# georghess/neurad-studio

Measured on AMD Instinct MI355X. Metric: ray-samples/sec (4096 rays x 128 samples), higher is better.
Workload: dtype f32; 1 GPU; BASELINE config[1]: NeuRAD hash-grid (16 levels, T=2^19, F=2, fp32) + 64-wide MLPs, 4096 rays x 128 samples per GPU, PowerSampler bins + ray ordering pass + fused field + compositing (forward / render path); rays_per_gpu=4096, samples_per_ray=128, parallelism=rays sharded x1, no collective

## Files before the change

### neurad_studio_amd/csrc/render.hip

```cpp
#include "common.h"
#include "render_variants.h"

namespace nrhip {

struct FieldDev {
  GridDev grid;
  const void* table;
  float scale;
  const float* gw0; const float* gb0;
  const float* gw1; const float* gb1;
  const float* fw0; const float* fb0;
  const float* fw1; const float* fb1;
  const float* fw2; const float* fb2;
  int use_sdf;
  float beta;
  uint32_t lay[NRHIP_MAX_LEVELS * 4];
};

struct SaveDev {
  float* enc;
  float* hg;
  float* xf;
  float* hf;
};
// ... 152 lines not shown
    d16[blk * 8 + 4 + v] = (unsigned short)(m >> 16);
    d16[NBLK * KB * 64 * 8 + blk * 4 + v] = (unsigned short)(l >> 16);
  }
}

using f16x8 = __attribute__((ext_vector_type(8))) _Float16;
using f16x2 = __attribute__((ext_vector_type(2))) _Float16;
using f32x2 = __attribute__((ext_vector_type(2))) float;
constexpr float kPairAct = 64.f, kPairW = 128.f, kPairFit = 65000.f;
constexpr bool kPairsDefault = true;

template <bool CHAIN, int NBLK, int KQ>
__device__ __forceinline__ float pair_src(const float* __restrict__ W, int ldw, int row_off, int e) {
  const int t = e & 7, lane = (e >> 3) & 63, rest = e >> 9;
  const int q = rest % KQ, mb = rest / KQ;
  const int i = lane & 15, g = lane >> 4;
  const int col = CHAIN ? (16 * (2 * q + (t >> 2)) + 4 * g + (t & 3)) : (8 * g + t);
  return W[(size_t)(row_off + 16 * mb + i) * ldw + col];
}
__device__ __forceinline__ bool pair_store(float* __restrict__ region, int N, int e, float w) {
  _Float16* d16 = reinterpret_cast<_Float16*>(region);
  const float ws = w * kPairW;
  const _Float16 h = (_Float16)ws;
  d16[e] = h;
  d16[N + e] = (_Float16)(ws - (float)h);
  return !(fabsf(ws) < kPairFit);
}

template <bool CHAIN, int NBLK, int KQ>
__device__ __forceinline__ void mfma_layer_pairs(const float* __restrict__ wf, const float* __restrict__ W, int ldw,
                                                 int row_off, bool wbad, int lane, const float (&b)[8 * KQ],
                                                 f32x4 (&acc)[NBLK]) {
  float mx = 0.f;
#pragma unroll
  for (int k = 0; k < 8 * KQ; ++k) mx = fmaxf(mx, fabsf(b[k]));
  if (__builtin_expect(wbad || __builtin_amdgcn_ballot_w64(!(mx < kPairFit)) != 0ull, 0)) {
    int opaque = 0;
    asm volatile("" : "+v"(opaque));
    const int g = lane >> 4;
    const float* Wl = W + (size_t)(row_off + (lane & 15)) * ldw + opaque;
#pragma unroll
    for (int s = 0; s < 8 * KQ; ++s) {
      const int col = CHAIN ? (16 * (s >> 2) + 4 * g + (s & 3)) : (8 * g + s);
#pragma unroll
      for (int mb = 0; mb < NBLK; ++mb)
        acc[mb] = __builtin_amdgcn_mfma_f32_16x16x4f32(Wl[(size_t)16 * mb * ldw + col] * kPairW, b[s], acc[mb], 0, 0, 0);
    }
  } else {
    const f16x8* w8 = reinterpret_cast<const f16x8*>(wf);
    constexpr int LO = NBLK * KQ * 64;
#pragma unroll
    for (int q = 0; q < KQ; ++q) {
      f16x8 xh, xl;
#pragma unroll
      for (int k = 0; k < 8; k += 2) {
        const f32x2 v = {b[8 * q + k], b[8 * q + k + 1]};
        const f16x2 h = __builtin_convertvector(v, f16x2);
        const f16x2 l = __builtin_convertvector(v - __builtin_convertvector(h, f32x2), f16x2);
        xh[k] = h[0], xh[k + 1] = h[1], xl[k] = l[0], xl[k + 1] = l[1];
      }
#pragma unroll
      for (int mb = 0; mb < NBLK; ++mb)
        acc[mb] = __builtin_amdgcn_mfma_f32_16x16x32_f16(w8[(mb * KQ + q) * 64 + lane], xh, acc[mb], 0, 0, 0);
#pragma unroll
      for (int mb = 0; mb < NBLK; ++mb)
        acc[mb] = __builtin_amdgcn_mfma_f32_16x16x32_f16(w8[LO + (mb * KQ + q) * 64 + lane], xh, acc[mb], 0, 0, 0);
#pragma unroll
      for (int mb = 0; mb < NBLK; ++mb)
        acc[mb] = __builtin_amdgcn_mfma_f32_16x16x32_f16(w8[(mb * KQ + q) * 64 + lane], xl, acc[mb], 0, 0, 0);
    }
  }
#pragma unroll
  for (int mb = 0; mb < NBLK; ++mb) acc[mb] *= 1.f / kPairW;
}

template <Prod PROD, bool CHAIN, int NBLK, int K>
__device__ __forceinline__ void tile_layer(const float* __restrict__ wf, const float* __restrict__ W, int ldw, int row_off,
                                           bool wbad, int lane, const float (&b)[K], f32x4 (&acc)[NBLK]) {
  if constexpr (PROD == Prod::F16Pairs) mfma_layer_pairs<CHAIN, NBLK, K / 8>(wf, W, ldw, row_off, wbad, lane, b, acc);
  else if constexpr (PROD == Prod::Bf16Split) mfma_layer_split<NBLK, K / 4>(wf, lane, b, acc);
  else mfma_layer<NBLK, K>(wf, lane, b, acc);
}

template <int L, int F, int H, Prod PROD = Prod::F32>
__device__ __forceinline__ void stage_field_weights(const FieldDev& fd, float* __restrict__ lds) {
  using Ld = Lds<H, PROD>;
  constexpr int LF = EncFrame<L, F>::LF;
  static_assert(PROD == Prod::F32 || EncFrame<L, F>::FULL, "split / pair products: L * F == 32 only");
  constexpr int NB = H / 16;
  constexpr int T = 256;
  constexpr int N_G0 = H * 32 / T, N_G1 = 32 * H / T, N_F0 = H * 32 / T, N_F1 = H * H / T, N_F2 = 32 * H / T,
                N_SH = 16 * H / T;
  static_assert((H * 32) % T == 0 && (H * H) % T == 0 && (16 * H) % T == 0, "regions are whole passes of the block");
  const int tid = threadIdx.x;
  float vg0[N_G0], vg1[N_G1], vf0[N_F0], vf1[N_F1], vf2[N_F2], vsh[N_SH], vs[7];
  if constexpr (PROD == Prod::Bf16Split) {
    stage_split_matrix<false, NB, 2>(lds + Ld::G0, fd.gw0, LF, 0);
    stage_split_matrix<true, 2, NB>(lds + Ld::G1, fd.gw1, H, 1);
    stage_split_matrix<true, NB, 2>(lds + Ld::F0, fd.fw0, 48, 0);
    stage_split_matrix<true, NB, NB>(lds + Ld::F1, fd.fw1, H, 0);
  } else if constexpr (PROD == Prod::F16Pairs) {
    static_assert(H % 32 == 0, "fp16 pairs: K = 32 steps");
    if (tid == 0) reinterpret_cast<int*>(lds)[Ld::FLG] = 0;
    __syncthreads();
#pragma unroll
    for (int it = 0; it < N_G0; ++it) vg0[it] = pair_src<false, NB, 1>(fd.gw0, LF, 0, it * T + tid);
#pragma unroll
    for (int it = 0; it < N_G1; ++it) vg1[it] = pair_src<true, 2, H / 32>(fd.gw1, H, 1, it * T + tid);
#pragma unroll
    for (int it = 0; it < N_F0; ++it) vf0[it] = pair_src<true, NB, 1>(fd.fw0, 48, 0, it * T + tid);
#pragma unroll
    for (int it = 0; it < N_F1; ++it) vf1[it] = pair_src<true, NB, H / 32>(fd.fw1, H, 0, it * T + tid);
  } else {
#pragma unroll
    for (int it = 0; it < N_G0; ++it) vg0[it] = enc_frag_src<L, F, NB>(fd.gw0, it * T + tid);
#pragma unroll
    for (int it = 0; it < N_G1; ++it) vg1[it] = frag_src<true, 2, H / 4>(fd.gw1, H, 1, it * T + tid);
#pragma unroll
    for (int it = 0; it < N_F0; ++it) vf0[it] = frag_src<true, NB, 8>(fd.fw0, 48, 0, it * T + tid);
#pragma unroll
    for (int it = 0; it < N_F1; ++it) vf1[it] = frag_src<true, NB, H / 4>(fd.fw1, H, 0, it * T + tid);
  }
#pragma unroll
  for (int it = 0; it < N_F2; ++it) vf2[it] = frag_src<true, 2, H / 4>(fd.fw2, H, 0, it * T + tid);
#pragma unroll
  for (int it = 0; it < N_SH; ++it) {
    const int e = it * T + tid, c = e / H, n = e - c * H;
    vsh[it] = fd.fw0[(size_t)n * 48 + 32 + c];
  }
  const int th = tid < H ? tid : 0, t33 = tid < 33 ? tid : 0, t32 = tid & 31;
  vs[0] = fd.gw1[th];
  vs[1] = fd.gb0 ? fd.gb0[th] : 0.f;
  vs[2] = fd.fb0 ? fd.fb0[th] : 0.f;
  vs[3] = fd.fb1 ? fd.fb1[th] : 0.f;
  vs[4] = fd.gb1 ? fd.gb1[t33] : 0.f;
  vs[5] = fd.fb2 ? fd.fb2[t32] : 0.f;
  vs[6] = fd.grid.scal[t32];
  if constexpr (PROD == Prod::F16Pairs) {
    constexpr float kB = kPairAct * kPairW;
    vs[0] *= 1.f / kPairAct, vs[1] *= kB, vs[2] *= kB, vs[3] *= kB;
    if (t33 != 0) vs[4] *= kB;
#pragma unroll
    for (int it = 0; it < N_F2; ++it) vf2[it] *= 1.f / kPairAct;
#pragma unroll
    for (int it = 0; it < N_SH; ++it) vsh[it] *= kB;
    bool bad = false;
#pragma unroll
    for (int it = 0; it < N_G0; ++it) bad |= pair_store(lds + Ld::G0, H * 32, it * T + tid, vg0[it]);
#pragma unroll
    for (int it = 0; it < N_G1; ++it) bad |= pair_store(lds + Ld::G1, 32 * H, it * T + tid, vg1[it]);
#pragma unroll
    for (int it = 0; it < N_F0; ++it) bad |= pair_store(lds + Ld::F0, H * 32, it * T + tid, vf0[it]);
#pragma unroll
    for (int it = 0; it < N_F1; ++it) bad |= pair_store(lds + Ld::F1, H * H, it * T + tid, vf1[it]);
    if (bad) reinterpret_cast<int*>(lds)[Ld::FLG] = 1;
  }
  if constexpr (PROD == Prod::F32) {
#pragma unroll
    for (int it = 0; it < N_G0; ++it) lds[Ld::G0 + it * T + tid] = vg0[it];
#pragma unroll
    for (int it = 0; it < N_G1; ++it) lds[Ld::G1 + it * T + tid] = vg1[it];
#pragma unroll
    for (int it = 0; it < N_F0; ++it) lds[Ld::F0 + it * T + tid] = vf0[it];
#pragma unroll
    for (int it = 0; it < N_F1; ++it) lds[Ld::F1 + it * T + tid] = vf1[it];
  }
#pragma unroll
  for (int it = 0; it < N_F2; ++it) lds[Ld::F2 + it * T + tid] = vf2[it];
#pragma unroll
  for (int it = 0; it < N_SH; ++it) lds[Ld::SHW + it * T + tid] = vsh[it];
  if (tid < H) {
    lds[Ld::SDFW + tid] = vs[0];
    lds[Ld::BG0 + tid] = vs[1];
    lds[Ld::BF0 + tid] = vs[2];
    lds[Ld::BF1 + tid] = vs[3];
  }
  if (tid < 33) lds[Ld::BG1 + tid] = vs[4];
  if (tid < 32) {
    lds[Ld::BF2 + tid] = vs[5];
    lds[Ld::SCAL + tid] = vs[6];
  }
}

__device__ __forceinline__ void stream_store(float* p, f32x4 v) { __builtin_nontemporal_store(v, reinterpret_cast<f32x4*>(p)); }

template <int N>
__device__ __forceinline__ float row_shr(float v, float fill) {
  return dpp_row_shr<N>(v, fill);
}
__device__ __forceinline__ float row_sum16(float v) {
  v += __shfl_xor(v, 1, 64);
  v += __shfl_xor(v, 2, 64);
  v += __shfl_xor(v, 4, 64);
  v += __shfl_xor(v, 8, 64);
  return v;
}

template <int LPL, int F>
struct TileFetch {
  float fv[LPL][8][F];
  float x, y, z, std;
  float t0, t1;
};

struct RayRange {
  int64_t end;
  int S, stride;
};

struct PendingTile {
  int64_t pos;
  int64_t ray;
  int t;
  bool valid;
  float t0, t1;
  float ox, oy, oz, dx, dy, dz, area;
  int ncand;
};

__device__ __forceinline__ float from_lane(float v, int byte_addr) {
  return __builtin_bit_cast(float, __builtin_amdgcn_ds_bpermute(byte_addr, __builtin_bit_cast(int, v)));
}
__device__ __forceinline__ void put_block(float* geo, int lane, const SamplePos& p) {
  geo[lane] = p.x, geo[64 + lane] = p.y, geo[128 + lane] = p.z, geo[192 + lane] = p.std;
}
__device__ __forceinline__ SamplePos get_block(const float* geo, int src) {
  SamplePos p;
  p.x = geo[src], p.y = geo[64 + src], p.z = geo[128 + src], p.std = geo[192 + src];
  return p;
}

template <bool ACT>
__device__ __forceinline__ void fill_block(float* geo, float* ageo, int lane, const PendingTile& pt, float scale) {
  if constexpr (ACT) {
    const SamplePos gs = sample_gaussian(pt.ox, pt.oy, pt.oz, pt.dx, pt.dy, pt.dz, pt.area, pt.t0, pt.t1);
    put_block(ageo, lane, gs);
    put_block(geo, lane, contract_gaussian(gs.x, gs.y, gs.z, gs.std, scale));
  } else {
    put_block(geo, lane, sample_position(pt.ox, pt.oy, pt.oz, pt.dx, pt.dy, pt.dz, pt.area, pt.t0, pt.t1, scale));
  }
}

__device__ __forceinline__ void load_pending(PendingTile& p, int64_t pos, int t, const RayRange& rr, int lane,
                                             const int32_t* __restrict__ order, const float* __restrict__ ro,
                                             const float* __restrict__ rd, const float* __restrict__ rarea,
                                             const float* __restrict__ rstarts, const float* __restrict__ rends,
                                             const int32_t* __restrict__ cand_count = nullptr) {
  p.pos = pos, p.t = t, p.valid = pos < rr.end;
  const int64_t pc = p.valid ? pos : rr.end - 1;
  const int64_t ray = order ? (int64_t)order[pc] : pc;
  p.ray = ray;
  const int s = p.valid ? 64 * (t >> 2) + lane : lane;
  const int64_t si = ray * rr.stride + (s < rr.S ? s : rr.S - 1);
  if ((t & 3) == 0) {
    p.t0 = rstarts[si];
    p.t1 = rends[si];
  }
  p.ox = ro[3 * ray], p.oy = ro[3 * ray + 1], p.oz = ro[3 * ray + 2];
  p.dx = rd[3 * ray], p.dy = rd[3 * ray + 1], p.dz = rd[3 * ray + 2];
  p.area = rarea[ray];
  p.ncand = cand_count ? cand_count[ray] : 0;
}

__device__ __forceinline__ void load_pending_packed(PendingTile& p, int64_t pos, int t, const RayRange& rr, int lane,
                                                    const int32_t* __restrict__ order, const float* __restrict__ ro,
                                                    const float* __restrict__ rd, const float* __restrict__ rarea,
                                                    const float* __restrict__ rstarts, const float* __restrict__ rends,
                                                    const int64_t* __restrict__ segs, int& first, int& count,
                                                    const int32_t* __restrict__ cand_count = nullptr) {
  p.pos = pos, p.t = t, p.valid = pos < rr.end;
  const int64_t pc = p.valid ? pos : rr.end - 1;
  const int64_t ray = order ? (int64_t)order[pc] : pc;
  p.ray = ray;
  const int b = (int)segs[ray], n = (int)segs[ray + 1] - b;
  first = b, count = n;
  const int s = p.valid ? 64 * (t >> 2) + lane : lane;
  int si = b + (s < n ? s : n - 1);
  si = si < 0 ? 0 : si;
  si = si < rr.S ? si : rr.S - 1;
  if ((t & 3) == 0) {
    p.t0 = rstarts[si];
    p.t1 = rends[si];
  }
  p.ox = ro[3 * ray], p.oy = ro[3 * ray + 1], p.oz = ro[3 * ray + 2];
  p.dx = rd[3 * ray], p.dy = rd[3 * ray + 1], p.dz = rd[3 * ray + 2];
  p.area = rarea[ray];
  p.ncand = cand_count ? cand_count[ray] : 0;
}

__device__ __forceinline__ void layout_corners(float x, float y, float z, float scale, uint32_t my, uint32_t mz,
                                               uint32_t mask, uint32_t (&idx)[8]) {
  const float sx = __fmul_rn(x, scale), sy = __fmul_rn(y, scale), sz = __fmul_rn(z, scale);
  const uint32_t ifx = (uint32_t)(int)floorf(sx), ify = (uint32_t)(int)floorf(sy), ifz = (uint32_t)(int)floorf(sz);
  const uint32_t icx = (uint32_t)(int)ceilf(sx), icy = (uint32_t)(int)ceilf(sy), icz = (uint32_t)(int)ceilf(sz);
  const uint32_t hyc = icy * my, hyf = ify * my, hzc = icz * mz, hzf = ifz * mz;
  idx[0] = (icx ^ hyc ^ hzc) & mask;
  idx[1] = (icx ^ hyf ^ hzc) & mask;
  idx[2] = (ifx ^ hyf ^ hzc) & mask;
  idx[3] = (ifx ^ hyc ^ hzc) & mask;
  idx[4] = (icx ^ hyc ^ hzf) & mask;
  idx[5] = (icx ^ hyf ^ hzf) & mask;
  idx[6] = (ifx ^ hyf ^ hzf) & mask;
  idx[7] = (ifx ^ hyc ^ hzf) & mask;
}

template <int L, int F, bool HALF, bool RELAY = false>
__device__ __forceinline__ void issue_tile(const FieldDev& fd, const PendingTile& pt, int g, uint32_t mask,
                                           const float* scal_lds, TileFetch<EncFrame<L, F>::LPL, F>& tf,
                                           float* geo, int lane, const uint32_t* lay_lds = nullptr) {
  constexpr int LPL = EncFrame<L, F>::LPL;
  if ((pt.t & 3) == 0) fill_block<false>(geo, nullptr, lane, pt, fd.scale);
  const int src = 16 * (pt.t & 3) + (lane & 15);
  const SamplePos p = get_block(geo, src);
  tf.t0 = from_lane(pt.t0, src << 2);
  tf.t1 = from_lane(pt.t1, src << 2);
  if (!EncFrame<L, F>::busy(g)) return;
#pragma unroll
  for (int q = 0; q < LPL; ++q) {
    if constexpr (RELAY) {
      const uint4 ly = *reinterpret_cast<const uint4*>(lay_lds + 4 * q);
      uint32_t idx[8];
      layout_corners(p.x, p.y, p.z, scal_lds[q], ly.x, ly.y, ly.z, idx);
#pragma unroll
      for (int k = 0; k < 8; ++k) Entry<F, HALF>::load(fd.table, ly.w + idx[k], tf.fv[q][k]);
    } else {
      const Corners cs = hash_corners(p.x, p.y, p.z, scal_lds[q], mask);
#pragma unroll
      for (int k = 0; k < 8; ++k)
        Entry<F, HALF>::load(fd.table, ((uint32_t)(LPL * g + q) << fd.grid.log2T) + cs.idx[k], tf.fv[q][k]);
    }
  }
}

template <int L, int F, bool HALF>
__device__ __forceinline__ void issue_tile_actors(const FieldDev& fd, const ActorFieldDev& ad, const PendingTile& pt, int g,
                                                  uint32_t mask, const float* scal_lds, const float* ascal_lds,
                                                  const int32_t* __restrict__ cand_actor,
                                                  const float* __restrict__ cand_w2b, const float* __restrict__ bounds,
                                                  const void* const* __restrict__ tables,
                                                  TileFetch<EncFrame<L, F>::LPL, F>& tf, int& slot_out,
                                                  float* geo, float* ageo, int lane) {
  constexpr int LPL = EncFrame<L, F>::LPL;
  const bool busy = EncFrame<L, F>::busy(g);
  const int n = __builtin_amdgcn_readfirstlane(pt.ncand);
  const uint32_t row = (uint32_t)__builtin_amdgcn_readfirstlane((int)((uint32_t)pt.ray * (uint32_t)ad.K));
  if ((pt.t & 3) == 0) fill_block<true>(geo, ageo, lane, pt, fd.scale);
  const int src = 16 * (pt.t & 3) + (lane & 15);
  const SamplePos gs = get_block(ageo, src), ps = get_block(geo, src);
  tf.t0 = from_lane(pt.t0, src << 2);
  tf.t1 = from_lane(pt.t1, src << 2);
  int slot = -1;
  if (n > 0) {
    for (int c = 0; c < n; ++c) {
      const float* w = cand_w2b + (row + (uint32_t)c) * 12u;
// ... 61 lines not shown
    const float nn = sqrtf(ddx * ddx + ddy * ddy + ddz * ddz) + 1e-7f;
    if (mine) bx = ddx / nn, by = ddy / nn, bz = ddz / nn;
  }
  float sh[16];
  sh4((bx + 1.f) / 2.f, (by + 1.f) / 2.f, (bz + 1.f) / 2.f, sh);
#pragma unroll
  for (int c = 0; c < 16; ++c)
    if ((c >> 2) == g) shb[c & 3] = sh[c];
}

template <int L, int F>
__device__ __forceinline__ void blend_tile_actors(const TileFetch<EncFrame<L, F>::LPL, F>& tf, int slot, int g, int La,
                                                  const float* scal_lds, const float* ascal_lds, float (&feat)[8]) {
  using EF = EncFrame<L, F>;
  constexpr int LPL = EF::LPL;
  const bool in_box = slot >= 0;
#pragma unroll
  for (int q = 0; q < LPL; ++q) {
    const int lv = LPL * g + q, alv = lv < La ? lv : La - 1;
    const float sc = in_box ? ascal_lds[alv] : scal_lds[q];
    Corners c;
    const float sx = __fmul_rn(tf.x, sc), sy = __fmul_rn(tf.y, sc), sz = __fmul_rn(tf.z, sc);
    c.ox = __fsub_rn(sx, floorf(sx)), c.oy = __fsub_rn(sy, floorf(sy)), c.oz = __fsub_rn(sz, floorf(sz));
    float v[F];
    lerp_corners<F>(c, tf.fv[q], v);
    const float rw = (in_box && lv >= La) ? 0.f : rescale_weight(sc, tf.std);
#pragma unroll
    for (int f = 0; f < F; ++f) feat[q * F + f] = EF::busy(g) ? v[f] * rw : 0.f;
  }
#pragma unroll
  for (int k = EF::W; k < 8; ++k) feat[k] = 0.f;
}

template <int L, int F>
__device__ __forceinline__ void blend_tile(const TileFetch<EncFrame<L, F>::LPL, F>& tf, const SamplePos& p, int g,
                                           const float* scal_lds, float (&feat)[8]) {
  using EF = EncFrame<L, F>;
  constexpr int LPL = EF::LPL;
#pragma unroll
  for (int q = 0; q < LPL; ++q) {
    const float sc = scal_lds[q];
    Corners c;
    const float sx = __fmul_rn(p.x, sc), sy = __fmul_rn(p.y, sc), sz = __fmul_rn(p.z, sc);
    c.ox = __fsub_rn(sx, floorf(sx)), c.oy = __fsub_rn(sy, floorf(sy)), c.oz = __fsub_rn(sz, floorf(sz));
    float v[F];
    lerp_corners<F>(c, tf.fv[q], v);
    const float rw = rescale_weight(sc, p.std);
#pragma unroll
    for (int f = 0; f < F; ++f) feat[q * F + f] = EF::busy(g) ? v[f] * rw : 0.f;
  }
#pragma unroll
  for (int k = EF::W; k < 8; ++k) feat[k] = 0.f;
}

template <int L, int F, int H, bool HALF, Out OUT, Src SRC, Prod PROD, Lay LAY = Lay::Dense>
__global__ __launch_bounds__(256, 2) void render_kernel(
    FieldDev fd, int64_t n_rays, int S, int stride, const int32_t* __restrict__ order, const float* __restrict__ ro,
    const float* __restrict__ rd, const float* __restrict__ rarea, const float* __restrict__ rstarts,
    const float* __restrict__ rends, float* __restrict__ out_feat, float* __restrict__ out_depth,
    float* __restrict__ out_acc, float* __restrict__ out_w, float* __restrict__ out_sdf, float* __restrict__ out_alpha,
    SaveDev sv, float stop_eps, const int32_t* __restrict__ range, ActorFieldDev ad,
    const int32_t* __restrict__ cand_count,
    const int32_t* __restrict__ cand_actor, const float* __restrict__ cand_w2b, const float* __restrict__ bounds,
    const void* const* __restrict__ tables) {
  using EF = EncFrame<L, F>;
  static_assert(render_variant_ok(L, F, OUT, SRC, PROD, LAY), "not a legal variant: see render_variant_ok");
  static_assert(H % 16 == 0 && H >= 16 && H <= 128, "hidden width");
  constexpr bool COMPOSITE = OUT == Out::Composite;
  constexpr bool ACT = SRC == Src::Actors, RELAY = SRC == Src::EvalTable, OVR = SRC == Src::Overrides;
  constexpr bool PAIRS = PROD == Prod::F16Pairs;
  constexpr bool PACKED = LAY != Lay::Dense;
  const int64_t* const segs = LAY == Lay::PackedActors ? reinterpret_cast<const int64_t*>(sv.enc)
                                                       : reinterpret_cast<const int64_t*>(tables);
  const int32_t* const pcand = ACT ? cand_count : nullptr;
  const int32_t* const ovr_row = cand_count;
  const float* const ovr_rows = cand_w2b;
  const float* const ovr_dirs = bounds;
  using Ld = Lds<H, PROD>;
  constexpr int NB = H / 16;
  constexpr int LPL = EF::LPL;
  constexpr bool DEFER = COMPOSITE;
  extern __shared__ __attribute__((aligned(16))) float lds[];

  stage_field_weights<L, F, H, PROD>(fd, lds);
  if constexpr (ACT || OVR) {
    for (int e = threadIdx.x; e < 16 * H; e += 256) lds[Ld::SHF + e] = frag_src<true, NB, 4>(fd.fw0 + 32, 48, 0, e);
  }
  if constexpr (ACT) {
    if (threadIdx.x < ad.La) lds[Ld::ASCAL + threadIdx.x] = ad.scal[threadIdx.x];
  }
  if constexpr (RELAY) {
    if (threadIdx.x < 4 * L) reinterpret_cast<uint32_t*>(lds + Ld::LAY)[threadIdx.x] = fd.lay[threadIdx.x];
  }
  __syncthreads();
  bool wbad = false;
  if constexpr (PAIRS) wbad = __builtin_amdgcn_readfirstlane(reinterpret_cast<const int*>(lds)[Ld::FLG]) != 0;

  const int lane = threadIdx.x & 63;
  const int wid = __builtin_amdgcn_readfirstlane(threadIdx.x >> 6);
  const int j = lane & 15, g = lane >> 4;
  const uint32_t mask = (1u << fd.grid.log2T) - 1u;
  const int ntile = (S + 15) >> 4;

  const int nx = (int)gridDim.x < 8 ? (int)gridDim.x : 8;
  const int xcd = (int)blockIdx.x % nx, lb = (int)blockIdx.x / nx;
  const int nblk = ((int)gridDim.x - xcd + nx - 1) / nx;
  const int64_t first = range ? range[0] : 0, count = range ? range[1] - range[0] : n_rays;
  const int64_t lo = first + count * xcd / nx;
  const RayRange rr{first + count * (xcd + 1) / nx, S, stride};
  const int64_t pos_step = (int64_t)nblk * 4;

  const float* scal_l = lds + Ld::SCAL + LPL * g;
  const uint32_t* lay_l = reinterpret_cast<const uint32_t*>(lds + Ld::LAY) + 4 * LPL * g;
  float* rbw = lds + Ld::RB + wid * H;
  int64_t pos = lo + (int64_t)lb * 4 + wid;
  if (pos >= rr.end) return;
  int t = 0;
  TileFetch<LPL, F> tf;
  if constexpr (!EF::FULL) tf = TileFetch<LPL, F>{};
  int ta = -1;
  const float* ascal_l = lds + Ld::ASCAL;
  PendingTile q;
  float* geo_w = lds + Ld::GEO + wid * kBlockGeo;
  float* ageo_w = lds + (ACT ? Ld::AGEO : Ld::GEO) + wid * kBlockGeo;
  int qb = 0, qn = 0;
  auto tiles_of = [](int n) { return n > 16 ? (n + 15) >> 4 : 1; };
  if constexpr (PACKED) load_pending_packed(q, pos, 0, rr, lane, order, ro, rd, rarea, rstarts, rends, segs, qb, qn, pcand);
  else load_pending(q, pos, 0, rr, lane, order, ro, rd, rarea, rstarts, rends, cand_count);
  int64_t ray = q.ray;
  int cb = 0, cn = 0;
  if constexpr (PACKED) cb = qb, cn = qn;
  if constexpr (ACT) issue_tile_actors<L, F, HALF>(fd, ad, q, g, mask, scal_l, ascal_l, cand_actor, cand_w2b, bounds, tables, tf, ta, geo_w, ageo_w, lane);
  else issue_tile<L, F, HALF, RELAY>(fd, q, g, mask, scal_l, tf, geo_w, lane, lay_l);
  if constexpr (OVR && PACKED) ta = (q.valid && j < qn && qb + j >= 0 && qb + j < S) ? ovr_row[qb + j] : -1;
  else if constexpr (OVR) ta = (q.valid && j < S) ? ovr_row[q.ray * S + j] : -1;
  {
    const bool wrap = (PACKED ? tiles_of(cn) : ntile) == 1;
    if constexpr (PACKED) load_pending_packed(q, wrap ? pos + pos_step : pos, wrap ? 0 : 1, rr, lane, order, ro, rd, rarea, rstarts, rends, segs, qb, qn, pcand);
    else load_pending(q, wrap ? pos + pos_step : pos, wrap ? 0 : 1, rr, lane, order, ro, rd, rarea, rstarts, rends, cand_count);
  }

  f32x4 shq = f32x4{0.f, 0.f, 0.f, 0.f};
  float carry = 0.f, acc_w = 0.f, acc_d = 0.f;
  constexpr int NHA = DEFER ? H / 4 : 1;
  float ha[NHA];
  f32x4 fa[2];

  while (true) {
    if (t == 0) {
      const float dx = rd[3 * ray], dy = rd[3 * ray + 1], dz = rd[3 * ray + 2];
      float sh[16];
      sh4((dx + 1.f) / 2.f, (dy + 1.f) / 2.f, (dz + 1.f) / 2.f, sh);
      if constexpr (!COMPOSITE) {
#pragma unroll
        for (int c = 0; c < 16; ++c)
          if ((c >> 2) == g) shq[c & 3] = sh[c];
      }
      f32x4 rb[NB];
#pragma unroll
      for (int mb = 0; mb < NB; ++mb) rb[mb] = *reinterpret_cast<const f32x4*>(lds + Ld::BF0 + 16 * mb + 4 * g);
#pragma unroll
      for (int c = 0; c < 16; ++c)
#pragma unroll
        for (int mb = 0; mb < NB; ++mb) {
          const f32x4 w = *reinterpret_cast<const f32x4*>(lds + Ld::SHW + c * H + 16 * mb + 4 * g);
#pragma unroll
          for (int r = 0; r < 4; ++r) rb[mb][r] = fmaf(w[r], sh[c], rb[mb][r]);
        }
#pragma unroll
      for (int mb = 0; mb < NB; ++mb) *reinterpret_cast<f32x4*>(rbw + 16 * mb + 4 * g) = rb[mb];
      carry = COMPOSITE ? (fd.use_sdf ? 1.f : 0.f) : 0.f;
      acc_w = 0.f, acc_d = 0.f;
      fa[0] = fa[1] = f32x4{0.f, 0.f, 0.f, 0.f};
#pragma unroll
      for (int k = 0; k < NHA; ++k) ha[k] = 0.f;
    }

    int opaque = 0;
    asm volatile("" : "+v"(opaque));
    const float* lw = lds + opaque;
    const int s = 16 * t + j;
    const bool live = s < (PACKED ? cn : S);
    const float t0 = tf.t0, t1 = tf.t1;

    float feat[8];
    bool tile_hit = false;
    float shb[4] = {0.f, 0.f, 0.f, 0.f};
    if constexpr (ACT) {
      blend_tile_actors<L, F>(tf, ta, g, ad.La, scal_l, ascal_l, feat);
      tile_hit = __ballot(ta >= 0) != 0ull;
      if (tile_hit)
        actor_tile_sh(ta, (uint32_t)__builtin_amdgcn_readfirstlane((int)((uint32_t)ray * (uint32_t)ad.K)), g, rd[3 * ray],
                      rd[3 * ray + 1], rd[3 * ray + 2], cand_w2b, shb);
    } else {
      blend_tile<L, F>(tf, get_block(geo_w, 16 * (t & 3) + j), g, scal_l, feat);
      if constexpr (PAIRS) {
#pragma unroll
        for (int k = 0; k < 8; ++k) feat[k] *= kPairAct;
      }
      if constexpr (OVR) {
        tile_hit = __ballot(ta >= 0) != 0ull;
        if (tile_hit) {
          float bx = rd[3 * ray], by = rd[3 * ray + 1], bz = rd[3 * ray + 2];
          if (ta >= 0) {
            const float* rp = ovr_rows + (size_t)ta * EF::LF + EF::W * g;
            if constexpr (EF::FULL) {
              const f32x4 r0 = *reinterpret_cast<const f32x4*>(rp), r1 = *reinterpret_cast<const f32x4*>(rp + 4);
#pragma unroll
              for (int k = 0; k < 4; ++k) feat[k] = r0[k], feat[4 + k] = r1[k];
            } else if (EF::busy(g)) {
#pragma unroll
              for (int k = 0; k < EF::W; ++k) feat[k] = rp[k];
            }
            bx = ovr_dirs[3 * (size_t)ta], by = ovr_dirs[3 * (size_t)ta + 1], bz = ovr_dirs[3 * (size_t)ta + 2];
          }
          float sh[16];
          sh4((bx + 1.f) / 2.f, (by + 1.f) / 2.f, (bz + 1.f) / 2.f, sh);
#pragma unroll
          for (int c = 0; c < 16; ++c)
            if ((c >> 2) == g) shb[c & 3] = sh[c];
        }
      }
    }
    __builtin_amdgcn_sched_barrier(0);

    bool stop_here = false;
    if constexpr (COMPOSITE) {
      if (stop_eps > 0.f) {
        const float c = __builtin_bit_cast(float, __builtin_amdgcn_readfirstlane(__builtin_bit_cast(int, carry)));
        stop_here = fd.use_sdf ? (c < stop_eps) : (c > -__logf(stop_eps));
      }
    }
    const bool last_tile = t == (PACKED ? tiles_of(cn) : ntile) - 1;
    const bool ray_done = last_tile || stop_here;

    if (ray_done && q.valid && q.pos == pos) {
      if constexpr (PACKED) load_pending_packed(q, pos + pos_step, 0, rr, lane, order, ro, rd, rarea, rstarts, rends, segs, qb, qn, pcand);
      else load_pending(q, pos + pos_step, 0, rr, lane, order, ro, rd, rarea, rstarts, rends, cand_count);
    }
    const bool have_next = q.valid;
    const int64_t npos = q.pos, nray = q.ray;
    const int nt = q.t;
    int nb = 0, nn = 0;
    if constexpr (PACKED) nb = qb, nn = qn;
    if constexpr (ACT) issue_tile_actors<L, F, HALF>(fd, ad, q, g, mask, scal_l, ascal_l, cand_actor, cand_w2b, bounds, tables, tf, ta, geo_w, ageo_w, lane);
    else issue_tile<L, F, HALF, RELAY>(fd, q, g, mask, scal_l, tf, geo_w, lane, lay_l);
    if constexpr (OVR && PACKED) {
      const int s2 = 16 * q.t + j;
      ta = (q.valid && s2 < qn && qb + s2 >= 0 && qb + s2 < S) ? ovr_row[qb + s2] : -1;
    } else if constexpr (OVR) {
      ta = (q.valid && 16 * q.t + j < S) ? ovr_row[q.ray * S + 16 * q.t + j] : -1;
    }
    {
// ... 142 lines not shown
      f32x4 o[2];
#pragma unroll
      for (int mb = 0; mb < 2; ++mb) o[mb] = *reinterpret_cast<const f32x4*>(lw + Ld::BF2 + 16 * mb + 4 * g);
      mfma_layer<2, H / 4>(lw + Ld::F2, lane, hb, o);
      if constexpr (PAIRS) {
        o[0] += e[0] * (1.f / kPairAct);
        o[1] += e[1] * (1.f / kPairAct);
      } else {
        o[0] += e[0];
        o[1] += e[1];
      }
      if (live) {
        const int64_t si = PACKED ? (int64_t)cb + s : ray * S + s;
        float* fp = out_feat + si * 32;
        stream_store(fp + 4 * g, o[0]);
        stream_store(fp + 16 + 4 * g, o[1]);
        if (g == 0) {
          out_sdf[si] = sdf;
          out_alpha[si] = a_or_d;
        }
      }
    } else {
      float w, T;
      if (fd.use_sdf) {
        const float alpha = live ? a_or_d : 0.f;
        float incl = 1.f - alpha;
        incl *= row_shr<1>(incl, 1.f);
        incl *= row_shr<2>(incl, 1.f);
        incl *= row_shr<4>(incl, 1.f);
        incl *= row_shr<8>(incl, 1.f);
        const float excl = row_shr<1>(incl, 1.f);
        T = carry * excl;
        w = T * alpha;
        carry *= __shfl(incl, (lane & 48) | 15, 64);
      } else {
        const float sd = live ? a_or_d * (t1 - t0) : 0.f;
        float incl = sd;
        incl += row_shr<1>(incl, 0.f);
        incl += row_shr<2>(incl, 0.f);
        incl += row_shr<4>(incl, 0.f);
        incl += row_shr<8>(incl, 0.f);
        const float excl = row_shr<1>(incl, 0.f);
        T = expf(-(carry + excl));
        w = T * (1.f - expf(-sd));
        carry += __shfl(incl, (lane & 48) | 15, 64);
      }
      if (out_w && live && g == 0) out_w[PACKED ? (int64_t)cb + s : ray * S + s] = w;
      acc_w += w;
      if (PACKED || s < S - 1) acc_d += w * ((t0 + t1) / 2.f);
      float wf = w;
      float acc = 0.f;
      if (ray_done) {
        acc = row_sum16(acc_w);
        if constexpr (!PACKED) {
          if (last_tile && s == S - 1) wf += 1.f - acc;
        }
      }
#pragma unroll
      for (int k = 0; k < H / 4; ++k) ha[k] = fmaf(hb[k], wf, ha[k]);
#pragma unroll
      for (int r = 0; r < 4; ++r) {
        fa[0][r] = fmaf(e[0][r], wf, fa[0][r]);
        fa[1][r] = fmaf(e[1][r], wf, fa[1][r]);
      }

      if (ray_done) {
        const float dep = row_sum16(acc_d);
        if (!last_tile && out_w)
          for (int s2 = 16 * (t + 1) + lane; s2 < (PACKED ? cn : S); s2 += 64)
            out_w[(PACKED ? (int64_t)cb : ray * S) + s2] = 0.f;
        const float wsum = (!PACKED && last_tile) ? acc + (1.f - acc) : acc;
        f32x4 of2[2] = {f32x4{0.f, 0.f, 0.f, 0.f}, f32x4{0.f, 0.f, 0.f, 0.f}};
        mfma_layer<2, H / 4>(lw + Ld::F2, lane, ha, of2);
#pragma unroll
        for (int mb = 0; mb < 2; ++mb) {
          const f32x4 b2 = *reinterpret_cast<const f32x4*>(lw + Ld::BF2 + 16 * mb + 4 * g);
#pragma unroll
          for (int r = 0; r < 4; ++r) {
            const float es = PAIRS ? fa[mb][r] * (1.f / kPairAct) : fa[mb][r];
            of2[mb][r] = fmaf(b2[r], wsum, row_sum16(of2[mb][r] + es));
          }
        }
        if (j == 0) {
          float* fp = out_feat + ray * 32;
          *reinterpret_cast<f32x4*>(fp + 4 * g) = of2[0];
          *reinterpret_cast<f32x4*>(fp + 16 + 4 * g) = of2[1];
          if (g == 0) {
            out_acc[ray] = acc;
            out_depth[ray] = dep;
          }
        }
      }
    }

    if (!have_next) break;
    pos = npos, ray = nray, t = nt;
    if constexpr (PACKED) cb = nb, cn = nn;
  }
}

struct Variant {
  int L, F, H;
  Out out;
  Src src;
  Prod prod;
};
constexpr Variant kVariants[] = {
#define X(L_, F_, H_, O_, S_, P_) {L_, F_, H_, Out::O_, Src::S_, Prod::P_},
    NRHIP_RENDER_VARIANTS(X)
#undef X
};

static bool same(const Variant& a, const Variant& b) {
  return a.L == b.L && a.F == b.F && a.H == b.H && a.out == b.out && a.src == b.src && a.prod == b.prod;
}
static bool has_variant(const Variant& v) {
  for (const Variant& r : kVariants)
    if (same(r, v)) return true;
  return false;
}

static int validate_field(const nrhip_field* f) {
  NR_REQUIRE(f, NRHIP_ERR_INVALID_ARG, "field descriptor is NULL");
  if (int e = validate_grid(&f->grid)) return e;
  NR_REQUIRE(f->table && f->static_scale > 0.f, NRHIP_ERR_INVALID_ARG, "field: NULL table or non-positive scale");
  const nrhip_mlp& a = f->geo;
  const nrhip_mlp& b = f->feat;
  const int L = f->grid.num_levels, F = f->grid.n_features, in = L * F;
  NR_REQUIRE(has_variant({L, F, a.hidden_dim, Out::Composite, Src::Static, Prod::F32}), NRHIP_ERR_UNSUPPORTED,
             "fused field kernel: no instantiation for L=%d F=%d H=%d (the grids and hidden widths: csrc/render_variants.h); "
             "use the unfused ops",
             L, F, a.hidden_dim);
  NR_REQUIRE(a.num_layers == 2 && b.num_layers == 3 && a.in_dim == in && a.out_dim == 33 && b.in_dim == 48 &&
                 b.out_dim == 32 && a.hidden_dim == b.hidden_dim,
             NRHIP_ERR_UNSUPPORTED,
             "fused field kernel needs geo L*F->H->33 (2 layers, L*F=%d) and feat 48->H->H->32 (3 layers); use the "
             "unfused ops",
             in);
  for (int l = 0; l < 2; ++l) NR_REQUIRE(a.weight[l], NRHIP_ERR_INVALID_ARG, "geo weight %d is NULL", l);
  for (int l = 0; l < 3; ++l) NR_REQUIRE(b.weight[l], NRHIP_ERR_INVALID_ARG, "feat weight %d is NULL", l);
  return NRHIP_OK;
}

static FieldDev to_dev(const nrhip_field& f) {
  FieldDev d;
  d.grid = to_dev(f.grid);
  d.table = f.table;
  d.scale = f.static_scale;
  d.gw0 = f.geo.weight[0], d.gb0 = f.geo.bias[0];
  d.gw1 = f.geo.weight[1], d.gb1 = f.geo.bias[1];
  d.fw0 = f.feat.weight[0], d.fb0 = f.feat.bias[0];
  d.fw1 = f.feat.weight[1], d.fb1 = f.feat.bias[1];
  d.fw2 = f.feat.weight[2], d.fb2 = f.feat.bias[2];
  d.use_sdf = f.use_sdf;
  d.beta = f.beta;
  for (int i = 0; i < NRHIP_MAX_LEVELS * 4; ++i)
    d.lay[i] = (f.eval_table && f.eval_layout && i < 4 * f.grid.num_levels) ? f.eval_layout[i] : 0u;
  return d;
}

struct ActorLaunch {
  ActorFieldDev ad;
  const int32_t* cand_count;
  const int32_t* cand_actor;
  const float* cand_w2b;
  const float* bounds;
  const void* const* tables;
};
struct OverrideLaunch {
// ... 353 lines not shown
```

Before: 3.752 billion ray-samples/s.

## Overlap weight staging with first tile fetch and vectorize fp16-pair weight loads

Splits weight staging into a register load phase and a later LDS store phase, so the first tile's hash-grid gathers and pending-ray loads are issued before the weights are converted and written to shared memory. The fp16-pair path now loads weights as 16-byte vectors when the pointers are aligned, with the old scalar path kept as a fallback. The per-ray SH bias row is recomputed with one output per lane rather than replicated f32x4 work, and early-exit waves now join the barrier before returning. The cost is higher register pressure from holding the staged weights across the tile issue, which could lower occupancy.

```diff
diff --git a/neurad_studio_amd/csrc/render.hip b/neurad_studio_amd/csrc/render.hip
--- a/neurad_studio_amd/csrc/render.hip
+++ b/neurad_studio_amd/csrc/render.hip
@@ -258,104 +258,188 @@
   else mfma_layer<NBLK, K>(wf, lane, b, acc);
 }
 
-template <int L, int F, int H, Prod PROD = Prod::F32>
-__device__ __forceinline__ void stage_field_weights(const FieldDev& fd, float* __restrict__ lds) {
+template <bool CHAIN, int NBLK, int KQ>
+__device__ __forceinline__ void pair_slot_load(const float* __restrict__ W, int ldw, int row_off, int slot, f32x4 (&v)[2]) {
+  const int lane = slot & 63, rest = slot >> 6;
+  const int q = rest % KQ, mb = rest / KQ;
+  const int i = lane & 15, g = lane >> 4;
+  const float* p = W + (size_t)(row_off + 16 * mb + i) * ldw + (CHAIN ? 32 * q + 4 * g : 8 * g);
+  v[0] = *reinterpret_cast<const f32x4*>(p);
+  v[1] = *reinterpret_cast<const f32x4*>(p + (CHAIN ? 16 : 4));
+}
+__device__ __forceinline__ bool pair_slot_store(float* __restrict__ region, int N, int slot, const f32x4 (&v)[2]) {
+  f16x8 hi, lo;
+  bool bad = false;
+#pragma unroll
+  for (int k = 0; k < 8; ++k) {
+    const float ws = v[k >> 2][k & 3] * kPairW;
+    const _Float16 h = (_Float16)ws;
+    hi[k] = h;
+    lo[k] = (_Float16)(ws - (float)h);
+    bad |= !(fabsf(ws) < kPairFit);
+  }
+  f16x8* d = reinterpret_cast<f16x8*>(region);
+  d[slot] = hi;
+  d[N / 8 + slot] = lo;
+  return bad;
+}
+__device__ __forceinline__ bool aligned16(const void* p) { return (reinterpret_cast<uintptr_t>(p) & 15) == 0; }
+
+template <int H, Prod PROD>
+struct StagedWeights {
+  static constexpr int T = 256;
+  static constexpr bool PAIRS = PROD == Prod::F16Pairs, F32 = PROD == Prod::F32;
+  static constexpr int N_G0 = H * 32 / T, N_G1 = 32 * H / T, N_F0 = H * 32 / T, N_F1 = H * H / T, N_F2 = 32 * H / T,
+                       N_SH = 16 * H / T;
+  static_assert((H * 32) % T == 0 && (H * H) % T == 0 && (16 * H) % T == 0, "regions are whole passes of the block");
+  static constexpr int S_G0 = H * 4, S_G1 = 4 * H, S_F0 = H * 4, S_F1 = H * H / 8;
+  static constexpr int P_G0 = (S_G0 + T - 1) / T, P_G1 = (S_G1 + T - 1) / T, P_F0 = (S_F0 + T - 1) / T,
+                       P_F1 = (S_F1 + T - 1) / T;
+  float vg0[F32 ? N_G0 : 1], vg1[F32 ? N_G1 : 1], vf0[F32 ? N_F0 : 1], vf1[F32 ? N_F1 : 1];
+  f32x4 pg0[PAIRS ? P_G0 : 1][2], pg1[PAIRS ? P_G1 : 1][2], pf0[PAIRS ? P_F0 : 1][2], pf1[PAIRS ? P_F1 : 1][2];
+  float vf2[N_F2], vsh[N_SH], vs[6];
+  bool wide[4];
+};
+
+template <int L, int F, int H, Prod PROD>
+__device__ __forceinline__ void load_field_weights(const FieldDev& fd, StagedWeights<H, PROD>& w) {
+  using SW = StagedWeights<H, PROD>;
+  constexpr int LF = EncFrame<L, F>::LF;
+  static_assert(PROD == Prod::F32 || EncFrame<L, F>::FULL, "split / pair products: L * F == 32 only");
+  constexpr int NB = H / 16, T = SW::T;
+  const int tid = threadIdx.x;
+  if constexpr (PROD == Prod::F16Pairs) {
+    static_assert(H % 32 == 0, "fp16 pairs: K = 32 steps");
+    w.wide[0] = aligned16(fd.gw0), w.wide[1] = aligned16(fd.gw1), w.wide[2] = aligned16(fd.fw0), w.wide[3] = aligned16(fd.fw1);
+    if (w.wide[0]) {
+#pragma unroll
+      for (int it = 0; it < SW::P_G0; ++it)
+        if (SW::S_G0 % T == 0 || it * T + tid < SW::S_G0) pair_slot_load<false, NB, 1>(fd.gw0, LF, 0, it * T + tid, w.pg0[it]);
+    }
+    if (w.wide[1]) {
+#pragma unroll
+      for (int it = 0; it < SW::P_G1; ++it)
+        if (SW::S_G1 % T == 0 || it * T + tid < SW::S_G1) pair_slot_load<true, 2, H / 32>(fd.gw1, H, 1, it * T + tid, w.pg1[it]);
+    }
+    if (w.wide[2]) {
+#pragma unroll
+      for (int it = 0; it < SW::P_F0; ++it)
+        if (SW::S_F0 % T == 0 || it * T + tid < SW::S_F0) pair_slot_load<true, NB, 1>(fd.fw0, 48, 0, it * T + tid, w.pf0[it]);
+    }
+    if (w.wide[3]) {
+#pragma unroll
+      for (int it = 0; it < SW::P_F1; ++it)
+        if (SW::S_F1 % T == 0 || it * T + tid < SW::S_F1) pair_slot_load<true, NB, H / 32>(fd.fw1, H, 0, it * T + tid, w.pf1[it]);
+    }
+  } else if constexpr (PROD == Prod::F32) {
+#pragma unroll
+    for (int it = 0; it < SW::N_G0; ++it) w.vg0[it] = enc_frag_src<L, F, NB>(fd.gw0, it * T + tid);
+#pragma unroll
+    for (int it = 0; it < SW::N_G1; ++it) w.vg1[it] = frag_src<true, 2, H / 4>(fd.gw1, H, 1, it * T + tid);
+#pragma unroll
+    for (int it = 0; it < SW::N_F0; ++it) w.vf0[it] = frag_src<true, NB, 8>(fd.fw0, 48, 0, it * T + tid);
+#pragma unroll
+    for (int it = 0; it < SW::N_F1; ++it) w.vf1[it] = frag_src<true, NB, H / 4>(fd.fw1, H, 0, it * T + tid);
+  }
+#pragma unroll
+  for (int it = 0; it < SW::N_F2; ++it) w.vf2[it] = frag_src<true, 2, H / 4>(fd.fw2, H, 0, it * T + tid);
+#pragma unroll
+  for (int it = 0; it < SW::N_SH; ++it) {
+    const int e = it * T + tid, c = e / H, n = e - c * H;
+    w.vsh[it] = fd.fw0[(size_t)n * 48 + 32 + c];
+  }
+  const int th = tid < H ? tid : 0, t33 = tid < 33 ? tid : 0, t32 = tid & 31;
+  w.vs[0] = fd.gw1[th];
+  auto bias = [&](const float* __restrict__ b, int i) {
+    const float v = (b ? b : fd.gw1)[i];
+    return b ? v : 0.f;
+  };
+  w.vs[1] = bias(fd.gb0, th);
+  w.vs[2] = bias(fd.fb0, th);
+  w.vs[3] = bias(fd.fb1, th);
+  w.vs[4] = bias(fd.gb1, t33);
+  w.vs[5] = bias(fd.fb2, t32);
+}
+
+template <int L, int F, int H, Prod PROD>
+__device__ __forceinline__ void store_field_weights(const FieldDev& fd, float* __restrict__ lds, StagedWeights<H, PROD>& w) {
+  using SW = StagedWeights<H, PROD>;
   using Ld = Lds<H, PROD>;
   constexpr int LF = EncFrame<L, F>::LF;
-  static_assert(PROD == Prod::F32 || EncFrame<L, F>::FULL, "split / pair products: L * F == 32 only");
-  constexpr int NB = H / 16;
-  constexpr int T = 256;
-  constexpr int N_G0 = H * 32 / T, N_G1 = 32 * H / T, N_F0 = H * 32 / T, N_F1 = H * H / T, N_F2 = 32 * H / T,
-                N_SH = 16 * H / T;
-  static_assert((H * 32) % T == 0 && (H * H) % T == 0 && (16 * H) % T == 0, "regions are whole passes of the block");
+  constexpr int NB = H / 16, T = SW::T;
   const int tid = threadIdx.x;
-  float vg0[N_G0], vg1[N_G1], vf0[N_F0], vf1[N_F1], vf2[N_F2], vsh[N_SH], vs[7];
+  const int t33 = tid < 33 ? tid : 0;
   if constexpr (PROD == Prod::Bf16Split) {
     stage_split_matrix<false, NB, 2>(lds + Ld::G0, fd.gw0, LF, 0);
     stage_split_matrix<true, 2, NB>(lds + Ld::G1, fd.gw1, H, 1);
     stage_split_matrix<true, NB, 2>(lds + Ld::F0, fd.fw0, 48, 0);
     stage_split_matrix<true, NB, NB>(lds + Ld::F1, fd.fw1, H, 0);
-  } else if constexpr (PROD == Prod::F16Pairs) {
-    static_assert(H % 32 == 0, "fp16 pairs: K = 32 steps");
-    if (tid == 0) reinterpret_cast<int*>(lds)[Ld::FLG] = 0;
-    __syncthreads();
-#pragma unroll
-    for (int it = 0; it < N_G0; ++it) vg0[it] = pair_src<false, NB, 1>(fd.gw0, LF, 0, it * T + tid);
-#pragma unroll
-    for (int it = 0; it < N_G1; ++it) vg1[it] = pair_src<true, 2, H / 32>(fd.gw1, H, 1, it * T + tid);
-#pragma unroll
-    for (int it = 0; it < N_F0; ++it) vf0[it] = pair_src<true, NB, 1>(fd.fw0, 48, 0, it * T + tid);
-#pragma unroll
-    for (int it = 0; it < N_F1; ++it) vf1[it] = pair_src<true, NB, H / 32>(fd.fw1, H, 0, it * T + tid);
-  } else {
-#pragma unroll
-    for (int it = 0; it < N_G0; ++it) vg0[it] = enc_frag_src<L, F, NB>(fd.gw0, it * T + tid);
-#pragma unroll
-    for (int it = 0; it < N_G1; ++it) vg1[it] = frag_src<true, 2, H / 4>(fd.gw1, H, 1, it * T + tid);
-#pragma unroll
-    for (int it = 0; it < N_F0; ++it) vf0[it] = frag_src<true, NB, 8>(fd.fw0, 48, 0, it * T + tid);
-#pragma unroll
-    for (int it = 0; it < N_F1; ++it) vf1[it] = frag_src<true, NB, H / 4>(fd.fw1, H, 0, it * T + tid);
-  }
-#pragma unroll
-  for (int it = 0; it < N_F2; ++it) vf2[it] = frag_src<true, 2, H / 4>(fd.fw2, H, 0, it * T + tid);
-#pragma unroll
-  for (int it = 0; it < N_SH; ++it) {
-    const int e = it * T + tid, c = e / H, n = e - c * H;
-    vsh[it] = fd.fw0[(size_t)n * 48 + 32 + c];
-  }
-  const int th = tid < H ? tid : 0, t33 = tid < 33 ? tid : 0, t32 = tid & 31;
-  vs[0] = fd.gw1[th];
-  vs[1] = fd.gb0 ? fd.gb0[th] : 0.f;
-  vs[2] = fd.fb0 ? fd.fb0[th] : 0.f;
-  vs[3] = fd.fb1 ? fd.fb1[th] : 0.f;
-  vs[4] = fd.gb1 ? fd.gb1[t33] : 0.f;
-  vs[5] = fd.fb2 ? fd.fb2[t32] : 0.f;
-  vs[6] = fd.grid.scal[t32];
+  }
   if constexpr (PROD == Prod::F16Pairs) {
     constexpr float kB = kPairAct * kPairW;
-    vs[0] *= 1.f / kPairAct, vs[1] *= kB, vs[2] *= kB, vs[3] *= kB;
-    if (t33 != 0) vs[4] *= kB;
-#pragma unroll
-    for (int it = 0; it < N_F2; ++it) vf2[it] *= 1.f / kPairAct;
-#pragma unroll
-    for (int it = 0; it < N_SH; ++it) vsh[it] *= kB;
+    w.vs[0] *= 1.f / kPairAct, w.vs[1] *= kB, w.vs[2] *= kB, w.vs[3] *= kB;
+    if (t33 != 0) w.vs[4] *= kB;
+#pragma unroll
+    for (int it = 0; it < SW::N_F2; ++it) w.vf2[it] *= 1.f / kPairAct;
+#pragma unroll
+    for (int it = 0; it < SW::N_SH; ++it) w.vsh[it] *= kB;
     bool bad = false;
-#pragma unroll
-    for (int it = 0; it < N_G0; ++it) bad |= pair_store(lds + Ld::G0, H * 32, it * T + tid, vg0[it]);
-#pragma unroll
-    for (int it = 0; it < N_G1; ++it) bad |= pair_store(lds + Ld::G1, 32 * H, it * T + tid, vg1[it]);
-#pragma unroll
-    for (int it = 0; it < N_F0; ++it) bad |= pair_store(lds + Ld::F0, H * 32, it * T + tid, vf0[it]);
-#pragma unroll
-    for (int it = 0; it < N_F1; ++it) bad |= pair_store(lds + Ld::F1, H * H, it * T + tid, vf1[it]);
+    if (w.wide[0]) {
+#pragma unroll
+      for (int it = 0; it < SW::P_G0; ++it)
+        if (SW::S_G0 % T == 0 || it * T + tid < SW::S_G0) bad |= pair_slot_store(lds + Ld::G0, H * 32, it * T + tid, w.pg0[it]);
+    } else {
+      for (int it = 0; it < SW::N_G0; ++it)
+        bad |= pair_store(lds + Ld::G0, H * 32, it * T + tid, pair_src<false, NB, 1>(fd.gw0, LF, 0, it * T + tid));
+    }
+    if (w.wide[1]) {
+#pragma unroll
+      for (int it = 0; it < SW::P_G1; ++it)
+        if (SW::S_G1 % T == 0 || it * T + tid < SW::S_G1) bad |= pair_slot_store(lds + Ld::G1, 32 * H, it * T + tid, w.pg1[it]);
+    } else {
+      for (int it = 0; it < SW::N_G1; ++it)
+        bad |= pair_store(lds + Ld::G1, 32 * H, it * T + tid, pair_src<true, 2, H / 32>(fd.gw1, H, 1, it * T + tid));
+    }
+    if (w.wide[2]) {
+#pragma unroll
+      for (int it = 0; it < SW::P_F0; ++it)
+        if (SW::S_F0 % T == 0 || it * T + tid < SW::S_F0) bad |= pair_slot_store(lds + Ld::F0, H * 32, it * T + tid, w.pf0[it]);
+    } else {
+      for (int it = 0; it < SW::N_F0; ++it)
+        bad |= pair_store(lds + Ld::F0, H * 32, it * T + tid, pair_src<true, NB, 1>(fd.fw0, 48, 0, it * T + tid));
+    }
+    if (w.wide[3]) {
+#pragma unroll
+      for (int it = 0; it < SW::P_F1; ++it)
+        if (SW::S_F1 % T == 0 || it * T + tid < SW::S_F1) bad |= pair_slot_store(lds + Ld::F1, H * H, it * T + tid, w.pf1[it]);
+    } else {
+      for (int it = 0; it < SW::N_F1; ++it)
+        bad |= pair_store(lds + Ld::F1, H * H, it * T + tid, pair_src<true, NB, H / 32>(fd.fw1, H, 0, it * T + tid));
+    }
     if (bad) reinterpret_cast<int*>(lds)[Ld::FLG] = 1;
   }
   if constexpr (PROD == Prod::F32) {
 #pragma unroll
-    for (int it = 0; it < N_G0; ++it) lds[Ld::G0 + it * T + tid] = vg0[it];
-#pragma unroll
-    for (int it = 0; it < N_G1; ++it) lds[Ld::G1 + it * T + tid] = vg1[it];
-#pragma unroll
-    for (int it = 0; it < N_F0; ++it) lds[Ld::F0 + it * T + tid] = vf0[it];
-#pragma unroll
-    for (int it = 0; it < N_F1; ++it) lds[Ld::F1 + it * T + tid] = vf1[it];
-  }
-#pragma unroll
-  for (int it = 0; it < N_F2; ++it) lds[Ld::F2 + it * T + tid] = vf2[it];
-#pragma unroll
-  for (int it = 0; it < N_SH; ++it) lds[Ld::SHW + it * T + tid] = vsh[it];
+    for (int it = 0; it < SW::N_G0; ++it) lds[Ld::G0 + it * T + tid] = w.vg0[it];
+#pragma unroll
+    for (int it = 0; it < SW::N_G1; ++it) lds[Ld::G1 + it * T + tid] = w.vg1[it];
+#pragma unroll
+    for (int it = 0; it < SW::N_F0; ++it) lds[Ld::F0 + it * T + tid] = w.vf0[it];
+#pragma unroll
+    for (int it = 0; it < SW::N_F1; ++it) lds[Ld::F1 + it * T + tid] = w.vf1[it];
+  }
+#pragma unroll
+  for (int it = 0; it < SW::N_F2; ++it) lds[Ld::F2 + it * T + tid] = w.vf2[it];
+#pragma unroll
+  for (int it = 0; it < SW::N_SH; ++it) lds[Ld::SHW + it * T + tid] = w.vsh[it];
   if (tid < H) {
-    lds[Ld::SDFW + tid] = vs[0];
-    lds[Ld::BG0 + tid] = vs[1];
-    lds[Ld::BF0 + tid] = vs[2];
-    lds[Ld::BF1 + tid] = vs[3];
-  }
-  if (tid < 33) lds[Ld::BG1 + tid] = vs[4];
-  if (tid < 32) {
-    lds[Ld::BF2 + tid] = vs[5];
-    lds[Ld::SCAL + tid] = vs[6];
-  }
+    lds[Ld::SDFW + tid] = w.vs[0];
+    lds[Ld::BG0 + tid] = w.vs[1];
+    lds[Ld::BF0 + tid] = w.vs[2];
+    lds[Ld::BF1 + tid] = w.vs[3];
+  }
+  if (tid < 33) lds[Ld::BG1 + tid] = w.vs[4];
+  if (tid < 32) lds[Ld::BF2 + tid] = w.vs[5];
 }
 
 __device__ __forceinline__ void stream_store(float* p, f32x4 v) { __builtin_nontemporal_store(v, reinterpret_cast<f32x4*>(p)); }
@@ -423,7 +507,7 @@
                                              const float* __restrict__ rstarts, const float* __restrict__ rends,
                                              const int32_t* __restrict__ cand_count = nullptr) {
   p.pos = pos, p.t = t, p.valid = pos < rr.end;
-  const int64_t pc = p.valid ? pos : rr.end - 1;
+  const int64_t pc = p.valid ? pos : (rr.end > 0 ? rr.end - 1 : 0);
   const int64_t ray = order ? (int64_t)order[pc] : pc;
   p.ray = ray;
   const int s = p.valid ? 64 * (t >> 2) + lane : lane;
@@ -445,7 +529,7 @@
                                                     const int64_t* __restrict__ segs, int& first, int& count,
                                                     const int32_t* __restrict__ cand_count = nullptr) {
   p.pos = pos, p.t = t, p.valid = pos < rr.end;
-  const int64_t pc = p.valid ? pos : rr.end - 1;
+  const int64_t pc = p.valid ? pos : (rr.end > 0 ? rr.end - 1 : 0);
   const int64_t ray = order ? (int64_t)order[pc] : pc;
   p.ray = ray;
   const int b = (int)segs[ray], n = (int)segs[ray + 1] - b;
@@ -673,19 +757,13 @@
   constexpr bool DEFER = COMPOSITE;
   extern __shared__ __attribute__((aligned(16))) float lds[];
 
-  stage_field_weights<L, F, H, PROD>(fd, lds);
-  if constexpr (ACT || OVR) {
-    for (int e = threadIdx.x; e < 16 * H; e += 256) lds[Ld::SHF + e] = frag_src<true, NB, 4>(fd.fw0 + 32, 48, 0, e);
-  }
-  if constexpr (ACT) {
-    if (threadIdx.x < ad.La) lds[Ld::ASCAL + threadIdx.x] = ad.scal[threadIdx.x];
-  }
-  if constexpr (RELAY) {
-    if (threadIdx.x < 4 * L) reinterpret_cast<uint32_t*>(lds + Ld::LAY)[threadIdx.x] = fd.lay[threadIdx.x];
-  }
-  __syncthreads();
-  bool wbad = false;
-  if constexpr (PAIRS) wbad = __builtin_amdgcn_readfirstlane(reinterpret_cast<const int*>(lds)[Ld::FLG]) != 0;
+  const float scal_v = fd.grid.scal[threadIdx.x & 31];
+  float ascal_v = 0.f;
+  uint32_t lay_v = 0u;
+  if constexpr (ACT) ascal_v = ad.scal[threadIdx.x & (NRHIP_MAX_LEVELS - 1)];
+  if constexpr (RELAY) lay_v = fd.lay[threadIdx.x & (4 * NRHIP_MAX_LEVELS - 1)];
+  StagedWeights<H, PROD> sw;
+  load_field_weights<L, F, H, PROD>(fd, sw);
 
   const int lane = threadIdx.x & 63;
   const int wid = __builtin_amdgcn_readfirstlane(threadIdx.x >> 6);
@@ -705,7 +783,7 @@
   const uint32_t* lay_l = reinterpret_cast<const uint32_t*>(lds + Ld::LAY) + 4 * LPL * g;
   float* rbw = lds + Ld::RB + wid * H;
   int64_t pos = lo + (int64_t)lb * 4 + wid;
-  if (pos >= rr.end) return;
+  const bool has_ray = pos < rr.end;
   int t = 0;
   TileFetch<LPL, F> tf;
   if constexpr (!EF::FULL) tf = TileFetch<LPL, F>{};
@@ -721,6 +799,17 @@
   int64_t ray = q.ray;
   int cb = 0, cn = 0;
   if constexpr (PACKED) cb = qb, cn = qn;
+  if (threadIdx.x < 32) lds[Ld::SCAL + threadIdx.x] = scal_v;
+  if constexpr (ACT) {
+    if (threadIdx.x < ad.La) lds[Ld::ASCAL + threadIdx.x] = ascal_v;
+  }
+  if constexpr (RELAY) {
+    if (threadIdx.x < 4 * L) reinterpret_cast<uint32_t*>(lds + Ld::LAY)[threadIdx.x] = lay_v;
+  }
+  if constexpr (PAIRS) {
+    if (threadIdx.x == 0) reinterpret_cast<int*>(lds)[Ld::FLG] = 0;
+  }
+  __syncthreads();
   if constexpr (ACT) issue_tile_actors<L, F, HALF>(fd, ad, q, g, mask, scal_l, ascal_l, cand_actor, cand_w2b, bounds, tables, tf, ta, geo_w, ageo_w, lane);
   else issue_tile<L, F, HALF, RELAY>(fd, q, g, mask, scal_l, tf, geo_w, lane, lay_l);
   if constexpr (OVR && PACKED) ta = (q.valid && j < qn && qb + j >= 0 && qb + j < S) ? ovr_row[qb + j] : -1;
@@ -730,6 +819,16 @@
     if constexpr (PACKED) load_pending_packed(q, wrap ? pos + pos_step : pos, wrap ? 0 : 1, rr, lane, order, ro, rd, rarea, rstarts, rends, segs, qb, qn, pcand);
     else load_pending(q, wrap ? pos + pos_step : pos, wrap ? 0 : 1, rr, lane, order, ro, rd, rarea, rstarts, rends, cand_count);
   }
+  __builtin_amdgcn_sched_barrier(0);
+
+  store_field_weights<L, F, H, PROD>(fd, lds, sw);
+  if constexpr (ACT || OVR) {
+    for (int e = threadIdx.x; e < 16 * H; e += 256) lds[Ld::SHF + e] = frag_src<true, NB, 4>(fd.fw0 + 32, 48, 0, e);
+  }
+  __syncthreads();
+  if (!has_ray) return;
+  bool wbad = false;
+  if constexpr (PAIRS) wbad = __builtin_amdgcn_readfirstlane(reinterpret_cast<const int*>(lds)[Ld::FLG]) != 0;
 
   f32x4 shq = f32x4{0.f, 0.f, 0.f, 0.f};
   float carry = 0.f, acc_w = 0.f, acc_d = 0.f;
@@ -747,19 +846,16 @@
         for (int c = 0; c < 16; ++c)
           if ((c >> 2) == g) shq[c & 3] = sh[c];
       }
-      f32x4 rb[NB];
-#pragma unroll
-      for (int mb = 0; mb < NB; ++mb) rb[mb] = *reinterpret_cast<const f32x4*>(lds + Ld::BF0 + 16 * mb + 4 * g);
-#pragma unroll
-      for (int c = 0; c < 16; ++c)
-#pragma unroll
-        for (int mb = 0; mb < NB; ++mb) {
-          const f32x4 w = *reinterpret_cast<const f32x4*>(lds + Ld::SHW + c * H + 16 * mb + 4 * g);
-#pragma unroll
-          for (int r = 0; r < 4; ++r) rb[mb][r] = fmaf(w[r], sh[c], rb[mb][r]);
+#pragma unroll
+      for (int n0 = 0; n0 < H; n0 += 64) {
+        const int n = n0 + lane;
+        if (H % 64 == 0 || n < H) {
+          float rb = lds[Ld::BF0 + n];
+#pragma unroll
+          for (int c = 0; c < 16; ++c) rb = fmaf(lds[Ld::SHW + c * H + n], sh[c], rb);
+          rbw[n] = rb;
         }
-#pragma unroll
-      for (int mb = 0; mb < NB; ++mb) *reinterpret_cast<f32x4*>(rbw + 16 * mb + 4 * g) = rb[mb];
+      }
       carry = COMPOSITE ? (fd.use_sdf ? 1.f : 0.f) : 0.f;
       acc_w = 0.f, acc_d = 0.f;
       fa[0] = fa[1] = f32x4{0.f, 0.f, 0.f, 0.f};
@@ -1068,9 +1164,11 @@
           }
         }
         if (j == 0) {
-          float* fp = out_feat + ray * 32;
-          *reinterpret_cast<f32x4*>(fp + 4 * g) = of2[0];
-          *reinterpret_cast<f32x4*>(fp + 16 + 4 * g) = of2[1];
+          int lane_o = lane;
+          asm volatile("" : "+v"(lane_o));
+          float* fp = out_feat + ray * 32 + 4 * (lane_o >> 4);
+          *reinterpret_cast<f32x4*>(fp) = of2[0];
+          *reinterpret_cast<f32x4*>(fp + 16) = of2[1];
           if (g == 0) {
             out_acc[ray] = acc;
             out_depth[ray] = dep;
```

After: 3.751 billion ray-samples/s. About the same (-0.0%).
